# mrnorman/miniWeatherML

Hardware: AMD Instinct MI355X
Metric: cell-updates/s (higher is better)
Workload: dtype f64; 1 GPU; supercell 400x400x100 nens=1 per GPU (global 400x400x100, dx = dy = 500 m), WENO-FV dycore only, 3 tracers, CFL dt; parallelism=1x1 slab, halo_transport=none, V=8, strict=0, weno_order=5, schedule=one stream, schedule_code=4, y_faces_in_one_launch=True, zero_tracer_shortcut=True, zero_stores_skipped=True, zero_row_maps=True, alg_bytes_per_cell_update=512, alg_bytes_per_cell_update_boundary=768

## Files before the change

include/mw_cdna4.h:

```cpp
#ifndef MW_CDNA4_H
#define MW_CDNA4_H

#ifdef __cplusplus
extern "C" {
#endif

#define MW_NUM_STATE 5
#define MW_MAX_TRACERS 16

enum { MW_DATA_THERMAL = 0, MW_DATA_SUPERCELL = 1, MW_DATA_CITY = 2, MW_DATA_BUILDING = 3 };
enum { MW_BC_PERIODIC = 0, MW_BC_OPEN = 1, MW_BC_WALL = 2 };

typedef struct {
  int nz, ny, nx, nens, num_tracers;
  long long nx_glob, ny_glob, i_beg, j_beg;
  double xlen, ylen, zlen;
  int px, py, nproc_x, nproc_y;
  int neigh[9];
  int bc_x, bc_y, bc_z;
  int use_immersed, enable_gravity;
  int idWV;
  double R_d, R_v, cp_d, cp_v, p0, grav, gamma_d, kappa_d, C0, earthrot, latitude;
} mw_grid_t;

// ... 40 lines not shown

int  mw_weno5_edges(long long n, const double *stencils, double *edges, int strict, void *stream);
int  mw_strict_pow(long long n, const double *x, const double *y, double *out, unsigned char *main_path, void *stream);

int  mw_calib_copy(const double *in, double *out, long long n, void *stream);

int  mw_calib_fma64(int waves_per_simd, double seconds, double *out5, void *stream);
long long mw_calib_stage_arith_threads(long long cells, int levels);
int  mw_calib_stage_arith(const double *tab, int nlev, long long cells, int levels, int active_tracers, const double *bg4, double *sink, double *out3, void *stream);
int  mw_debug_spin(long long usec, void *stream);
long long mw_debug_launched_kernels(char *buf, long long cap, int reset);
long long mw_debug_zero_maps(mw_dycore_t h, unsigned int *out_host, long long cap_words, int *dims2);
long long mw_debug_zero_violations(mw_dycore_t h, unsigned long long *out4);
long long mw_debug_vapour_redo(mw_dycore_t h);
long long mw_debug_tracer_flags(mw_dycore_t h, unsigned char *out_host, long long cap);

int  mw_perturb_temperature(const mw_grid_t *g, double *temp, void *stream);
int  mw_perturb_temperature_random(const mw_grid_t *g, double *temp, void *stream);

int  mw_exchange_plan(const mw_grid_t *g, int *peers, int *send_order, int *recv_order, int *active);
typedef int (*mw_exchange_fn)(void *ctx, const double *sendW, const double *sendE, const double *sendS,
                              const double *sendN, double *recvW, double *recvE, double *recvS, double *recvN,
                              long long nWE, long long nSN, void *stream);
int  mw_dycore_set_exchange(mw_dycore_t h, mw_exchange_fn fn, void *ctx);
int  mw_rccl_unique_id(unsigned char *id128);
int  mw_dycore_use_rccl(mw_dycore_t h, const unsigned char *id128, int nranks, int myrank);
int  mw_dycore_use_rccl_self(mw_dycore_t h);
const char *mw_rccl_library_path(int *version);
int  mw_dycore_rccl_info(mw_dycore_t h, int *comm_ranks, int *comm_rank, int *lanes);
int  mw_dycore_rccl_allreduce_sum(void *dycore_handle, double *buf, long long n, void *stream);
// ... 155 lines not shown
```

miniweatherml_amd/capi.py:

```python
import ctypes as C
import os

_HERE = os.path.dirname(os.path.abspath(__file__))
LIB_PATH = os.environ.get("MW_LIB_PATH") or os.path.join(_HERE, "libmw_cdna4.so")

MW_MAX_TRACERS = 16
MW_SURROGATE_MAX_MODELS = 256
MW_ROLLOUT_MAX_MEMBERS = 30
MW_COMMITTEE_MAX_MODELS = 16
MW_RAIN_MAX_FIELDS, MW_RAIN_MAX_THRESHOLDS = 4, 8
DATA_THERMAL, DATA_SUPERCELL, DATA_CITY, DATA_BUILDING = 0, 1, 2, 3
BC_PERIODIC, BC_OPEN, BC_WALL = 0, 1, 2
INIT_IDS = {"thermal": DATA_THERMAL, "supercell": DATA_SUPERCELL, "city": DATA_CITY, "building": DATA_BUILDING}


class Grid(C.Structure):
    _fields_ = [
        ("nz", C.c_int), ("ny", C.c_int), ("nx", C.c_int), ("nens", C.c_int), ("num_tracers", C.c_int),
        ("nx_glob", C.c_longlong), ("ny_glob", C.c_longlong), ("i_beg", C.c_longlong), ("j_beg", C.c_longlong),
        ("xlen", C.c_double), ("ylen", C.c_double), ("zlen", C.c_double),
        ("px", C.c_int), ("py", C.c_int), ("nproc_x", C.c_int), ("nproc_y", C.c_int),
        ("neigh", C.c_int * 9),
        ("bc_x", C.c_int), ("bc_y", C.c_int), ("bc_z", C.c_int),
        ("use_immersed", C.c_int), ("enable_gravity", C.c_int),
# ... 25 lines not shown
    "mw_dycore_set_bc": (C.c_int, [C.c_void_p, C.c_int, C.c_int, C.c_int]),
    "mw_dycore_set_strict": (C.c_int, [C.c_void_p, C.c_int]),
    "mw_dycore_set_order": (C.c_int, [C.c_void_p, C.c_int]),
    "mw_dycore_set_option": (C.c_int, [C.c_void_p, C.c_char_p, C.c_longlong]),
    "mw_dycore_get_option": (C.c_int, [C.c_void_p, C.c_char_p, C.POINTER(C.c_longlong)]),
    "mw_build_flags": (C.c_int, []),
    "mw_calib_fma64": (C.c_int, [C.c_int, C.c_double, C.POINTER(C.c_double), C.c_void_p]),
    "mw_calib_stage_arith_threads": (C.c_longlong, [C.c_longlong, C.c_int]),
    "mw_calib_stage_arith": (C.c_int, [C.c_void_p, C.c_int, C.c_longlong, C.c_int, C.c_int, C.POINTER(C.c_double), C.c_void_p, C.POINTER(C.c_double), C.c_void_p]),
    "mw_debug_spin": (C.c_int, [C.c_longlong, C.c_void_p]),
    "mw_debug_launched_kernels": (C.c_longlong, [C.c_char_p, C.c_longlong, C.c_int]),
    "mw_debug_zero_maps": (C.c_longlong, [C.c_void_p, C.c_void_p, C.c_longlong, C.POINTER(C.c_int)]),
    "mw_debug_zero_violations": (C.c_longlong, [C.c_void_p, C.POINTER(C.c_ulonglong)]),
    "mw_debug_vapour_redo": (C.c_longlong, [C.c_void_p]),
    "mw_debug_tracer_flags": (C.c_longlong, [C.c_void_p, C.c_void_p, C.c_longlong]),
    "mw_dycore_path": (C.c_char_p, [C.c_void_p]),
    "mw_dycore_use_rccl_self": (C.c_int, [C.c_void_p]),
    "mw_rccl_selftest_config": (C.c_int, [C.c_int, C.c_int]),
    "mw_dycore_time_step": (C.c_int, [C.c_void_p] + [C.c_void_p] * 5 + [C.POINTER(C.c_void_p), C.c_double]),
    "mw_dycore_compute_tendencies": (C.c_int, [C.c_void_p] + [C.c_void_p] * 5 + [C.POINTER(C.c_void_p), C.c_double,
                                                                               C.c_void_p, C.c_void_p]),
    "mw_dycore_get_fluxes": (C.c_int, [C.c_void_p, C.POINTER(C.c_void_p)]),
    "mw_dycore_get_etime": (C.c_double, [C.c_void_p]),
    "mw_dycore_schedule": (C.c_int, [C.c_void_p]),
    "mw_dycore_rccl_info": (C.c_int, [C.c_void_p, C.POINTER(C.c_int), C.POINTER(C.c_int), C.POINTER(C.c_int)]),
    "mw_dycore_rccl_allreduce_sum": (C.c_int, [C.c_void_p, C.c_void_p, C.c_longlong, C.c_void_p]),
    "mw_dycore_rccl_bcast": (C.c_int, [C.c_void_p, C.c_void_p, C.c_longlong, C.c_int, C.c_void_p]),
    "mw_dycore_profile": (C.c_int, [C.c_void_p, C.c_int]),
    "mw_dycore_profile_get": (C.c_int, [C.c_void_p, C.c_int, C.POINTER(C.c_double), C.POINTER(C.c_longlong)]),
    "mw_calib_copy": (C.c_int, [C.c_void_p, C.c_void_p, C.c_longlong, C.c_void_p]),
# ... 142 lines not shown
```

miniweatherml_amd/csrc/mw_dycore.hip:

```cpp
#include "mw_dycore_int.h"
#include "mw_weno.h"
#include <map>
#include <set>
#include <tuple>
#include <mutex>
#include <cmath>
#include <cstring>

namespace mw {
static std::mutex g_launch_mu;
static std::set<const void *> g_launched;
void note_launch(const void *fn) { std::lock_guard<std::mutex> lk(g_launch_mu); g_launched.insert(fn); }

__global__ __launch_bounds__(256) void k_coupler_to_state(DyP p, CouplerPtrs c, double *__restrict__ S) {
#pragma clang fp contract(off)
  long long t = (long long)blockIdx.x * 256 + threadIdx.x;
  int k = blockIdx.y;
  int NXI = p.nx * p.nens;
  if (t >= (long long)p.ny * NXI) return;
  int j = (int)(t / NXI), ie = (int)(t - (long long)j * NXI);
  int e = ie % p.nens;
  long long ci = ((long long)k * p.ny + j) * NXI + ie;
  double rho_d = c.rho_d[ci], u = c.u[ci], v = c.v[ci], w = c.w[ci], temp = c.temp[ci];
  double rho_v = c.tr[p.idWV][ci];
// ... 807 lines not shown
namespace {
struct OptDesc { const char *key; int DyOpts::*field; long long lo, hi; int build; };
const OptDesc OPTS[] = {
  {"overlap", &DyOpts::overlap, -1, 1, 0}, {"pipe", &DyOpts::pipe, 0, 1, 0}, {"pipe_edge_inline", &DyOpts::pipe_edge_inline, 0, 1, 0},
  {"pipe_convert", &DyOpts::pipe_convert, 0, 1, 0}, {"pipe_split_edges", &DyOpts::pipe_split_edges, 0, 1, 0}, {"spec", &DyOpts::spec, 0, 1, 0}, {"wrap", &DyOpts::wrap, 0, 1, 0},
  {"y_all", &DyOpts::y_all, 0, 1, 0}, {"y_all_conv", &DyOpts::y_all_conv, 0, 1, 0}, {"member_major", &DyOpts::member_major, 0, 1, 0},
  {"mm_direct", &DyOpts::mm_direct, 0, 1, 0}, {"mm_conv", &DyOpts::mm_conv, 0, 1, 0}, {"fused_convert", &DyOpts::fused_convert, 0, 1, 0},
  {"fused_convert_mm", &DyOpts::fused_convert_mm, 0, 1, 0}, {"chunk_y", &DyOpts::chunk_y, 0, 1 << 20, 0}, {"chunk_yt", &DyOpts::chunk_yt, 0, 1 << 20, 0},
  {"chunk_z", &DyOpts::chunk_z, 0, 1 << 20, 0}, {"chunk_f", &DyOpts::chunk_f, 0, 1 << 20, 0}, {"chunk_model", &DyOpts::chunk_model, 0, 1, 0},
  {"tf_rows4", &DyOpts::tf_rows4, 0, 1, 0}, {"zero_skip", &DyOpts::zero_skip, 0, 1, 0}, {"zero_rows", &DyOpts::zero_rows, 0, 1, 0}, {"zero_stores", &DyOpts::zero_stores, 0, 1, 0}, {"zero_verify", &DyOpts::zero_verify, 0, 1, 0}, {"pipe_maps_early", &DyOpts::pipe_maps_early, 0, 1, 0}, {"rccl_lanes", &DyOpts::rccl_lanes, 0, 2, 0}, {"rccl_two_comms", &DyOpts::rccl_two_comms, -1, 1, 0},
  {"xchg_fuzz", &DyOpts::xchg_fuzz, 0, 0x7fffffff, 0}, {"rccl_prio", &DyOpts::rccl_prio, 0, 1, 0}, {"rccl_inline", &DyOpts::rccl_inline, 0, 1, 0},
  {"debug_no_patch", &DyOpts::debug_no_patch, 0, 1, 0},
};
struct OptDesc2 { const char *key; int DyOpts::*field; };
const OptDesc2 OPTS_VAPOUR[] = {{"vapour_state", &DyOpts::vapour_state}, {"debug_vapour_redo", &DyOpts::debug_vapour_redo}};
constexpr int BUILD_FLAGS = 0;
}
int mw_build_flags(void) { return BUILD_FLAGS; }
int mw_dycore_set_option(mw_dycore_t d, const char *key, long long value) {
  if (!d || !key) MW_FAIL("mw_dycore_set_option: null argument");
  if (!strcmp(key, "fused_tracers")) {
    if (value != 0 && value != 1) MW_FAIL("option fused_tracers must be 0 or 1");
    if (value && !(d->g.num_tracers <= 4 && d->g.nens <= 12)) MW_FAIL("option fused_tracers = 1 needs at most 4 tracers and 12 members");
    d->fused = (int)value;
    return 0;
  }
  for (const OptDesc2 &od : OPTS_VAPOUR) {
    if (strcmp(key, od.key)) continue;
    if (value != 0 && value != 1) MW_FAIL(std::string("option ") + key + " must be 0 or 1");
    d->o.*(od.field) = (int)value;
    return 0;
  }
  for (const OptDesc &od : OPTS) {
    if (strcmp(key, od.key)) continue;
    if (value < od.lo || value > od.hi) MW_FAIL(std::string("option ") + key + ": value out of range [" + std::to_string(od.lo) + ", " + std::to_string(od.hi) + "]");
    d->o.*(od.field) = (int)value;
    if (!strncmp(key, "chunk_", 6)) d->chunk_y = d->chunk_yt = d->chunk_z = d->chunk_f = 0;
    return 0;
  }
  MW_FAIL(std::string("unknown option: ") + key);
}
int mw_dycore_get_option(mw_dycore_t d, const char *key, long long *value) {
  if (!d || !key || !value) MW_FAIL("mw_dycore_get_option: null argument");
  if (!strcmp(key, "fused_tracers")) { *value = d->fused; return 0; }
  for (const OptDesc2 &od : OPTS_VAPOUR) if (!strcmp(key, od.key)) { *value = d->o.*(od.field); return 0; }
  for (const OptDesc &od : OPTS) if (!strcmp(key, od.key)) { *value = d->o.*(od.field); return 0; }
  MW_FAIL(std::string("unknown option: ") + key);
}
int mw_dycore_set_order(mw_dycore_t d, int ord) {
  if (!d) MW_FAIL("null handle");
  if (ord != 3 && ord != 5 && ord != 7 && ord != 9) MW_FAIL("WENO order must be 3, 5, 7 or 9");
  const int hs = (ord - 1) / 2, hx = std::max(HXc, hs + 1), hz = std::max(HZc, hs);
  const int old_ord = d->ord, old_hx = d->hxw, old_hz = d->hzw;
  auto rollback = [&]() { d->ord = old_ord; d->hxw = old_hx; d->hzw = old_hz; fill_params(d); return 1; };
  d->ord = ord; d->hxw = hx; d->hzw = hz;
  fill_params(d);
  if (!d->strides_ok) { set_error("mw_dycore_set_order: with this order's halo a variable of the block has more than 2^31 - 1 elements"); return rollback(); }
  if (check_halo_fit(d)) return rollback();
  if (hx != old_hx || hz != old_hz) {
    MW_HIP(hipStreamSynchronize(d->stream));
// ... 315 lines not shown
```

miniweatherml_amd/csrc/mw_dycore_int.h:

```cpp
#pragma once
#include "mw_common.h"
#include "mw_zero_rows.h"
#include <string>
#include <vector>
#include <algorithm>

#pragma GCC visibility push(hidden)

namespace mw { void note_launch(const void *fn); }
#define MW_KLAUNCH(kern, ...) do { mw::note_launch((const void *)&kern); hipLaunchKernelGGL(kern, __VA_ARGS__); } while (0)

using namespace mw;

struct DyOpts {
  int overlap = -1;
  int pipe = 1;
  int pipe_edge_inline = 0;
  int pipe_convert = 1;
  int pipe_split_edges = 1;
  int spec = 1;
  int wrap = 1;
  int y_all = 1, y_all_conv = 1;
  int member_major = 1, mm_direct = 1, mm_conv = 1;
  int fused_convert = 1, fused_convert_mm = 1;
  int chunk_y = 0, chunk_yt = 0, chunk_z = 0, chunk_f = 0;
  int chunk_model = 1;
  int tf_rows4 = 1;
  int zero_skip = 1;
  int zero_rows = 1;
  int pipe_maps_early = 1;
  int zero_stores = 1;
  int zero_verify = 0;
  int rccl_lanes = 0, rccl_two_comms = -1;
  int rccl_prio = 1;
  int rccl_inline = 1;
  int xchg_fuzz = 0;
  int debug_no_patch = 0;
  int vapour_state = 1;
  int debug_vapour_redo = 0;
};

struct mw_dycore_s {
  mw_grid_t g;
  DyOpts o;
  unsigned char pos[MW_MAX_TRACERS], adds[MW_MAX_TRACERS];
  DyP p;
  bool strides_ok = true;
  int ord = 5;
  int hxw = HXc, hzw = HZc;
  double etime = 0;
  int strict = 0;
  int last_march = 0;
  std::string path;
  double *S0 = nullptr, *S1 = nullptr, *S2 = nullptr, *S3 = nullptr;
// ... 99 lines not shown
```

miniweatherml_amd/csrc/mw_march.h:

```cpp
#pragma once
#include "mw_zero_rows.h"
#ifndef MW_XCD_SWIZZLE
#define MW_XCD_SWIZZLE 1
#endif

namespace mw {

__device__ __forceinline__ double shfl_from(double v, int src_lane) { return __shfl(v, src_lane, 64); }

__device__ __forceinline__ double fast_rcp(double x) {
#pragma clang fp contract(fast)
  double r = __builtin_amdgcn_rcp(x);
  r = r + r * (1.0 - x * r);
  r = r + r * (1.0 - x * r);
  return r;
}

#define MW_SCHED_FENCE() __builtin_amdgcn_sched_barrier(0)

template <int N>
__device__ __forceinline__ void landed(double (&a)[N]) {
#pragma unroll
  for (int i = 0; i < N; i++) asm volatile("" : "+v"(a[i]));
}
// ... 742 lines not shown
  return qnew;
}
__device__ __forceinline__ double tr_times(double a, double b) {
#pragma clang fp contract(off)
  return a * b;
}
__device__ __forceinline__ double tr_d13_temp(double press, double rho_dry, double rho_v, double R_d, double R_v) {
#pragma clang fp contract(off)
  return press / (rho_dry * R_d + rho_v * R_v);
}
struct XzVap {
  const double *FY;
  double *cq;
  double *crho, *ctemp;
  unsigned *redo;
};


template <int STAGE, bool N1, int MODE, int HPL, int K, int ORD, bool MT = false, bool VAP = false>
__global__ __launch_bounds__(256, 2) void k_xz_state(DyP p, const double *__restrict__ S, const double *__restrict__ Sn,
                                                  double *__restrict__ Sout, double *__restrict__ MX, double *__restrict__ MZ,
                                                  unsigned char *__restrict__ UPX, unsigned char *__restrict__ UPZ,
                                                  const double *__restrict__ tendY, double dt_stage, double dt_dyn, int chunk,
                                                  int tiles_x, double *__restrict__ cu, double *__restrict__ cv, double *__restrict__ cw,
                                                  MemberOff mo, XzVap va) {
  static_assert(!MT || (N1 && HPL && MODE == 1), "the member-co-located form is the D13 variant of the nens == 1 kernel");
  static_assert(!VAP || (N1 && HPL && K == 1 && !MT && ORD == 5), "the vapour form exists for the folded supercell configuration with nens == 1, WENO-5");
  constexpr int HS = (ORD - 1) / 2;
  const int wv = __builtin_amdgcn_readfirstlane((int)(threadIdx.x >> 6));
  int mt_e = 0, mt_sub = 0;
  if (MT) {
    mt_e = wv & (mo.n - 1); mt_sub = wv >> mo.sh;
    S += mt_e * mo.slab; Sn += mt_e * mo.slab; Sout += mt_e * mo.slab; MX += mt_e * mo.mx; UPX += mt_e * mo.mx; MZ += mt_e * mo.mz; UPZ += mt_e * mo.mz;
    tendY += mt_e * mo.tend; p.hypk += mt_e * mo.per; p.ce = mt_e;
  }
  __shared__ double lds_c[8];
  __shared__ double lds_xpart[5][256], lds_fzprev[5][256];
  extern __shared__ double lds_hp_all[];
  Segment sg;
  block_segment(chunk, p.nz, sg);
  const XzGeom g = xz_geom<N1, ORD>(p, sg.col, sg.a, sg.b, tiles_x, 0, MT ? mt_sub : -1, MT ? 4 >> mo.sh : 4);
  const int seg_len = sg.b - sg.a;
  double *lds_hp = lds_hp_all + (MT ? wv * (seg_len + 2) * 8 : 0);
// ... 12 lines not shown
  double *lds_q = lds_hp_all + (chunk + 2) * 8 + threadIdx.x;
  const int n = g.n, lane = g.lane, NXI = g.NXI, j = g.j, q = g.q, e = g.e;
  const double *col = S + (long long)(j + p.HY) * p.sJ + (long long)p.HX * n + g.qa;
  const long long cell0 = (long long)j * NXI + g.qc;
  const long long slab0 = (long long)(j + p.HY) * p.sJ + (long long)p.HX * n + g.qc;
  const int planeC = p.ny * NXI;
  double w[5][ORD], nxt[5], ct[5];
#pragma unroll
  for (int v = 0; v < 5; v++) {
    ct[v] = 0; lds_fzprev[v][threadIdx.x] = 0; lds_xpart[v][threadIdx.x] = 0;
#pragma unroll
    for (int s = 0; s < ORD; s++) w[v][s] = load_zlevel<K>(p, col + (long long)v * p.sV, g.kstart - HS + s, v == idW);
  }
  const bool vzq_on = VAP && MODE == 1 && (p.zq != nullptr) && p.zero_skip;
  unsigned vzseg = 0;
  if (VAP && MODE == 1) { const int tx_ = (q + (HS + 1) - lane) ; vzseg = zr_seg_mask(tx_ - (HS + 2), tx_ - (HS + 1) + 63 + 1, NXI, p.wrap_x != 0); }
  unsigned long long vlean_mask = 0ull;
  auto vlean_fetch = [&](int kc0) __attribute__((always_inline)) {
    const unsigned wz = p.zq[(long long)min(kc0 + lane + 2, p.nz - 1) * p.zq_ld + j + MW_ZR_HALO];
    vlean_mask = __ballot((wz & vzseg) == 0u);
  };
  if (VAP && MODE == 1 && vzq_on) vlean_fetch(g.ka);
  double wq[ORD], nxtq = 0, ctq = 0;
  int qr = (g.kstart - HS + ORD) % ORD;
#define MW_QSLOT(s_) (lds_q[(5 + ((qr + (s_)) >= ORD ? qr + (s_) - ORD : qr + (s_))) * 256])
  if (VAP) {
    lds_q[0] = 0; lds_q[256] = 0; lds_q[512] = 0; lds_q[768] = 0; lds_q[1024] = 0;
#pragma unroll
    for (int s = 0; s < ORD; s++) wq[s] = load_zlevel<K>(p, col + (long long)5 * p.sV, g.kstart - HS + s, false);
  }
#pragma unroll
  for (int v = 0; v < 5; v++) landed(w[v]);
  if (VAP) landed(wq);
  if (VAP) {
#pragma unroll
    for (int s = 0; s < ORD; s++) MW_QSLOT(s) = wq[s];
  }
  for (int k = g.kstart; k <= g.kb; k++) {
    const bool top = (k == p.nz);
    const bool xwork = (k >= g.ka) && (k < g.kb);
    const bool zface = (k >= g.ka);
    const bool fin = (k > g.ka);
    bool vlean = false;
    if (VAP && MODE == 1 && vzq_on) {
      const int ic = max(k - 1, g.ka) - g.ka;
      if (ic > 0 && (ic & 63) == 0) vlean_fetch(g.ka + ic);
      vlean = (vlean_mask >> (ic & 63)) & 1ull;
    }
    {
      const int kn = min(k + HS + 1, p.nz + p.HZ - 1);
#pragma unroll
      for (int v = 0; v < 5; v++) nxt[v] = load_zlevel<K>(p, col + (long long)v * p.sV, kn, v == idW);
      if (VAP) nxtq = load_zlevel<K>(p, col + (long long)5 * p.sV, kn, false);
    }
    double snv[5], tyv[5], immv = 0;
    const int kfc = max(k - 1, g.ka), kxc = min(max(k, g.ka), g.kb - 1);
#pragma unroll
    for (int l = 0; l < 5; l++) { snv[l] = 0; tyv[l] = 0; }
    if (STAGE != 1) {
#pragma unroll
      for (int l = 0; l < 5; l++) snv[l] = Sn[(long long)l * p.sV + slab0 + (long long)(kfc + p.HZ) * p.sK];
    }
// ... 89 lines not shown
        for (int s = 0; s < ORD; s++) wq[s] = MW_QSLOT(s);
        double beq; weno_window_edges<ORD>(wq, beq, teq); fzq = fs.m_upw * (up ? beq : ctq);
      }
      upz = up;
    }
    landed(nxt); landed(snv); landed(tyv); landed(immv);
    if (VAP) {
      landed(nxtq); landed(qnv); landed(fysq); landed(fynq);
      if (!top) MW_QSLOT(0) = nxtq;
      if (xwork) {
        const double feq = from_east<N1>(fxq, lane, n);
        lds_q[(k & 1) * 256] = tr_partial_xy(feq, fxq, fynq, fysq, lds_c[0], lds_c[4]);
        lds_q[(2 + (k & 1)) * 256] = tr_out_xy(tr_out_pair(feq, fxq, lds_c[0]), tr_out_pair(fynq, fysq, lds_c[4]));
      }
    }
    if (xwork && g.owns_face && (g.owns_cell || q >= NXI)) {
      const long long fo = (long long)k * p.fxK + (long long)j * p.fxJ + q;
      MX[fo] = fxs[idR];  UPX[fo] = (unsigned char)upx;
    }
    if (zface && g.owns_cell) {
      const long long fo = (long long)k * p.fzK + (long long)j * p.fzJ + q;
      MZ[fo] = fzs[idR];  UPZ[fo] = (unsigned char)upz;
    }
    if (fin) {
      const int kc = k - 1;
      const double hyc = HPL ? lds_hp[(kc - g.kstart) * 8] : p.hypk[(long long)(kc * n + e) * 8];
      constexpr int wi = HS - 1;
      const double rho_s = w[idR][wi] + hyc;
      const double rho_n = (STAGE == 1) ? rho_s : snv[idR] + hyc;
      double imm_coef = 0;
      if (Cf<K>::immersed(p)) { double tau = 1.e3 * dt_stage; imm_coef = -fmin(1.0, dt_stage / tau); }
      const double ru_s = w[idU][wi] * rho_s, rv_s = w[idV][wi] * rho_s;
      double inv_rho_new = 1.0;
      double *so = Sout + slab0 + (long long)(kc + p.HZ) * p.sK;
      double xpart[5], fzprev[5];
// ... 15 lines not shown
        if (l == idV && Cf<K>::sim2d(p)) tend = 0;
        if (Cf<K>::immersed(p)) { double imm_tend = imm_coef * q_s / dt_stage; tend = immv * imm_tend + (1 - immv) * tend; }
        double qnew;
        const double cdt = HPL ? lds_c[2] : (STAGE == 1) ? dt_dyn : (STAGE == 2) ? (1.0 / 4.0) * dt_dyn : (2.0 / 3.0) * dt_dyn;
        if (STAGE == 1)      qnew = q_n + cdt * tend;
        else if (STAGE == 2) qnew = (3.0 / 4.0) * q_n + (1.0 / 4.0) * q_s + cdt * tend;
        else                 qnew = (1.0 / 3.0) * q_n + (2.0 / 3.0) * q_s + cdt * tend;
        if (l == idR) inv_rho_new = fast_rcp(qnew + hyc);
        if (VAP && MODE == 1 && l == idR) rho_new_q = qnew + hyc;
        double stored = (l == idR || l == idT) ? qnew : qnew * inv_rho_new;
        if (MODE == 1 && l == idT) {
          const double *hq = HPL ? lds_hp + (kc - g.kstart) * 8 : p.hypk + (long long)(kc * n + e) * 8;
          stored = pressure_fast<K>(p, qnew, hq[1], hq[2], hq[3]);
          if (VAP) press_q = stored;
        }
        if (g.owns_cell && !(MODE == 1 && (l == idU || l == idV || l == idW))) so[(long long)l * p.sV] = stored;
        if (MODE == 1 && g.owns_cell && (l == idU || l == idV || l == idW))
          (l == idU ? cu : l == idV ? cv : cw)[cpl(p, cell0 + (long long)kc * planeC)] = stored;
      }
      if (VAP) {
        const double qs_raw = MW_QSLOT(wi);
        const double mass_available = tr_mass_available(qs_raw, rho_s);
        const double mass_out = tr_mass_out(oxyq, tr_out_pair(fzq, fzpq, lds_c[1]), lds_c[5]);
        if (__builtin_expect(g.owns_cell && mass_out > mass_available, 0)) *va.redo = 1u;
        const double q_s = tr_times(qs_raw, rho_s);
        const double q_n = (STAGE == 1) ? q_s : tr_times(qnv, rho_n);
        const double qnew = tr_combine<STAGE>(q_n, q_s, tr_tend(Pq, fzq, fzpq, lds_c[1]), lds_c[2], true);
        if (g.owns_cell) {
          if (MODE == 0) so[(long long)5 * p.sV] = tr_times(qnew, inv_rho_new);
          else           va.cq[cpl(p, cell0 + (long long)kc * planeC)] = qnew;
          if (MODE == 1 && vlean) {
// ... 205 lines not shown
    c.temp[ci] = press / (rho_dry * p.R_d + rho_v * p.R_v);
  }
}

template <int STAGE, int MODE, int T, bool N1, int K, int ORD, bool MT = false, int VS = 0>
__global__ __launch_bounds__(256, 2) void k_tracers_fused(DyP p, const double *__restrict__ S, const double *__restrict__ Sn, double *Sout,
                                                       const double *__restrict__ FY, const double *__restrict__ MX,
                                                       const double *__restrict__ MZ, const unsigned char *__restrict__ UPX,
                                                       const unsigned char *__restrict__ UPZ, double *__restrict__ DS,
                                                       double *__restrict__ DN, unsigned char *__restrict__ flags, unsigned int *__restrict__ dirty,
                                                       double dt, double dt_dyn, CouplerPtrs c, int chunk, int tiles_x, int rows4, MemberOff mo,
                                                       unsigned *vr, int vslot) {
  static_assert(N1 || ORD == 5, "the neighbour-load form exists for WENO-5 only");
  static_assert(!VS || (N1 && K == 1 && T == 3 && !MT && ORD == 5), "the form without the vapour exists for the folded supercell configuration with nens == 1, WENO-5");
  bool vredo = true;
  if (VS) {
    vredo = __builtin_amdgcn_readfirstlane((int)vr[vslot]) != 0;
    if (blockIdx.x == 0 && blockIdx.y == 0 && threadIdx.x == 0) { vr[(vslot + 1) & 7] = 0u; if (vredo) atomicAdd(&vr[8], 1u); }
  }
  static_assert(!MT || (N1 && MODE == 1), "the member-co-located form (see MemberOff) is the D13 variant of the nens == 1 kernel");
  constexpr int HS = (ORD - 1) / 2;
  const int wv = __builtin_amdgcn_readfirstlane((int)(threadIdx.x >> 6));
  int mt_e = 0, mt_sub = 0;
  if (MT) {
    mt_e = wv & (mo.n - 1); mt_sub = wv >> mo.sh;
    S += mt_e * mo.slab; Sn += mt_e * mo.slab; Sout += mt_e * mo.slab; FY += mt_e * mo.fy; MX += mt_e * mo.mx; UPX += mt_e * mo.mx;
    MZ += mt_e * mo.mz; UPZ += mt_e * mo.mz; DS += mt_e * mo.fx; DN += mt_e * mo.fz; flags += mt_e * mo.cells;
    p.hyc += mt_e * mo.per; p.ce = mt_e;
  }
  const int n = N1 ? 1 : p.nens;
  constexpr int t0 = 0;
// ... 40 lines not shown
  const int k_lo = max(ka - 1, 0);
  const int k_hi = min(kb, p.nz - 1);
  const int kstart = max(ka - 2, 0);
#if MW_ZERO_SKIP
  if (VS && !vredo && (p.zq != nullptr) && p.zero_skip && kb + 1 - kstart < 64) {
    const unsigned zseg_ = zr_seg_mask(tx * U - (hw + 1) * n, tx * U - hw * n + 63 + n, NXI, p.wrap_x != 0);
    const int kit = kstart + lane;
    const bool in_it = kit <= kb + 1, st_it = (kit - 2 >= ka) && (kit - 2 < kb);
    bool busy = in_it && (p.zq[(long long)min(kit, p.nz - 1) * p.zq_ld + j + MW_ZR_HALO] & zseg_) != 0u;
    const unsigned *zc_ = (MODE == 1) ? p.zqc : p.zqp;
    if (zc_ != nullptr) {
      const int kq_ = (MODE == 1) ? min(max(kit - 2, ka), kb - 1) : min(kit, p.nz - 1);
      busy = busy || (st_it && (zc_[(long long)kq_ * p.zq_ld + j + MW_ZR_HALO] & zseg_) != 0u);
    } else busy = true;
    if (!__any(busy)) {
      if (upd && do_y) for (int kp = ka; kp < kb; kp++) flags[(long long)(kp * p.ny + j) * NXI + q] = (unsigned char)0;
      return;
    }
  }
#endif
  double w[T][ORD], nxt[T], ct[T];
  double fxp[T], fzp[T], multp[T], szf[T], P[T];
  double wkm2[T];
  double rhos2 = 0;

#pragma unroll
  for (int v = 0; v < T; v++) {
    ct[v] = 0; fxp[v] = fzp[v] = szf[v] = P[v] = 0; multp[v] = 1; wkm2[v] = 0;
#pragma unroll
    for (int s = 0; s < ORD; s++) w[v][s] = load_zlevel(p, col + (long long)v * p.sV, kstart - HS + s, false);
  }
// ... 337 lines not shown
```

miniweatherml_amd/csrc/mw_march_sched.hip:

```cpp
#include "mw_dycore_int.h"
#include "mw_weno.h"
#define MW_MARCH_SCHED_KERNELS
#include "mw_march.h"

template <int STAGE, int MODE>
static int rk_stage_march(mw_dycore_s *d, double *Sin, const double *Sn, double *Sout, double dt_stage, double dt_dyn,
                          const CouplerPtrs &c) {
  const long long gs = d->gstage++;
  const int par = (int)(gs & 1), slot = (int)(gs & 7);
  hipStream_t ss = d->stream, ts = d->overlap ? d->tstream : d->stream;
  const int T = d->p.nt;
  zero_rows_stage(d, STAGE);
  ProfScope stage_scope(d, 8, ss);
  if (d->overlap && gs >= 2) MW_HIP(hipStreamWaitEvent(ss, d->ev_tr[(gs - 2) & 7], 0));
  if (halo_fill(d, Sin, 0, 5, ss, 0, true)) return 1;
  const bool conv = (STAGE == 1) && d->conv_pending;
  d->conv_pending = false;
  const bool mm_conv_ok = d->mm_direct && d->o.mm_conv && marching_config(d, view(d, 0).p) != 0;
  const bool yall = y_all_ok(d) && !(conv && ((d->member_major && !mm_conv_ok) || !d->o.y_all_conv));
  if (STAGE == 1) { if (conv) zero_rows_conv(d, Sin, false, ss); else zero_rows_forget(d, Sin); }
  if (STAGE == 3 && MODE == 0) zero_rows_forget(d, Sout);
  const bool vap = yall && d->o.vapour_state && d->fused && !d->overlap && !d->member_major && d->p.nens == 1 && d->ord == 5 && marching_config(d, d->p) == 1;
  const int vap_slot = vap ? slot : -1;
  {
// ... 151 lines not shown
    MW_KLAUNCH(k_coupler_to_state_fast, s ? plane_grid(nstrip, p.nz) : cgrid, dim3(256), 0, d->stream, p, c, d->S0, ylo, yhi, s ? 1 : 0);
  }
  MW_LAUNCH_CHECK();
  return 0;
}

extern "C" {
long long mw_debug_tracer_flags(mw_dycore_t d, unsigned char *out_host, long long cap) {
  if (!d || !d->flags) return -1;
  (void)hipStreamSynchronize(d->stream);
  if (d->tstream) (void)hipStreamSynchronize(d->tstream);
  const long long n = (long long)d->p.nC;
  if (out_host && cap > 0 && hipMemcpy(out_host, d->flags, (size_t)std::min(n, cap), hipMemcpyDeviceToHost) != hipSuccess) return -1;
  return n;
}
long long mw_debug_vapour_redo(mw_dycore_t d) {
  if (!d || !d->dirty) return -1;
  (void)hipStreamSynchronize(d->stream);
  if (d->tstream) (void)hipStreamSynchronize(d->tstream);
  unsigned int n = 0;
  if (hipMemcpy(&n, d->dirty + MW_VREDO_RING + 8, sizeof(n), hipMemcpyDeviceToHost) != hipSuccess) return -1;
  return (long long)n;
}
}
```

miniweatherml_amd/csrc/mw_march_tracers.hip:

```cpp
#include "mw_dycore_int.h"
#include "mw_weno.h"
#include "mw_march.h"

template <int T, bool N1>
static void launch_xz_tracers_t(mw_dycore_s *d, const double *S, dim3 grid, int chunk, int tiles_x, int t0, int par, double dt, int rows4,
                                hipStream_t st) {
  MW_KLAUNCH((k_xz_tracers<T, N1>), grid, dim3(256), 0, st, d->p, S, d->FX, d->FY, d->FZ, d->M[par][0], d->M[par][2], d->UP[par][0],
                     d->UP[par][2], dt, chunk, tiles_x, t0, rows4);
}

int launch_xz_tracers(mw_dycore_s *d, const double *S, int par, double dt, hipStream_t st) {
  const DyP &p = d->p;
  ProfScope ps(d, 7, st);
  dim3 grid; int chunk, tiles_x;
  if (xz_grid(d, p, grid, chunk, tiles_x)) return 1;
  const int rows4 = p.ny >= 4 ? 1 : 0;
  if (rows4) grid.x = (unsigned)(((p.ny + 3) / 4) * tiles_x);
  for (int t0 = 0; t0 < p.nt; t0 += 4) {
    int cnt = std::min(4, p.nt - t0);
    if (p.nens == 1) {
      switch (cnt) { case 1: launch_xz_tracers_t<1, true>(d, S, grid, chunk, tiles_x, t0, par, dt, rows4, st); break;
                     case 2: launch_xz_tracers_t<2, true>(d, S, grid, chunk, tiles_x, t0, par, dt, rows4, st); break;
                     case 3: launch_xz_tracers_t<3, true>(d, S, grid, chunk, tiles_x, t0, par, dt, rows4, st); break;
                     default: launch_xz_tracers_t<4, true>(d, S, grid, chunk, tiles_x, t0, par, dt, rows4, st); break; }
// ... 11 lines not shown
template <int STAGE, int MODE>
int launch_tracer_update(mw_dycore_s *d, const double *Sstar, const double *Sn, double *Sout, double dt_dyn, const CouplerPtrs &c,
                                hipStream_t st) {
  ProfScope ps(d, 2, st);
  const DyP &p = d->p;
  dim3 grid = plane_grid((long long)p.ny * p.nx * p.nens, p.nz);
  MW_KLAUNCH((k_tracer_update<STAGE, MODE>), grid, dim3(256), 0, st, p, Sstar, Sn, Sout, d->FX, d->FY, d->FZ, dt_dyn, c);
  MW_LAUNCH_CHECK();
  return 0;
}

template <int STAGE, int MODE, int T, bool N1, int K, int ORD = 5, int VS = 0>
static void launch_tracers_fused_t(mw_dycore_s *d, const View &v, const double *S, const double *Sn, double *Sout, dim3 grid, int chunk, int tiles_x, int par,
                                   double dt, double dt_dyn, const CouplerPtrs &c, int rows4, hipStream_t st, int vap_slot) {
  const int e = v.e;
  MW_KLAUNCH((k_tracers_fused<STAGE, MODE, T, N1, K, ORD, false, VS>), grid, dim3(256), 0, st, v.p, v.S(S), v.S(Sn), v.S(Sout), d->FY + e * v.f[1],
                     d->M[par][0] + e * v.m[0], d->M[par][2] + e * v.m[2], d->UP[par][0] + e * v.m[0], d->UP[par][2] + e * v.m[2],
                     d->FX + e * v.f[0], d->FZ + e * v.f[2], d->flags + e * v.cells, d->dirty + (d->fused_launches & 1), dt, dt_dyn, c, chunk, tiles_x, rows4, MemberOff(),
                     VS ? d->dirty + MW_VREDO_RING : nullptr, VS ? vap_slot : 0);
}
template <int STAGE, int MODE>
int launch_tracers_fused(mw_dycore_s *d, const double *S, const double *Sn, double *Sout, int par, double dt, double dt_dyn,
                                const CouplerPtrs &c, hipStream_t st, int vap_slot) {
  {
    ProfScope ps(d, 7, st);
    bool direct = false;
    if constexpr (STAGE == 3 && MODE == 1) direct = d->mm_direct;
    if constexpr (STAGE == 3 && MODE == 1) if (direct) {
      const View v = view(d, 0);
      const DyP &p = v.p;
      const MemberOff mo = member_off(d);
      const int U = 64 - 2 * ((d->ord - 1) / 2 + 1), tiles_x = (p.nx + U - 1) / U, rpb = 4 / mo.n;
      const long long waves = (long long)p.ny * tiles_x;
      const int chunk = d->chunk_f ? d->chunk_f : (d->chunk_f = balanced_chunk(d, p.nz, waves, d->o.chunk_f, 10000, 2, 4.5, true));
// ... 64 lines not shown
```

miniweatherml_amd/csrc/mw_march_xz.hip:

```cpp
#include "mw_dycore_int.h"
#include "mw_weno.h"
#include "mw_march.h"

int xz_grid(mw_dycore_s *d, const DyP &p, dim3 &grid, int &chunk, int &tiles_x) {
  int U = xz_cells_per_wave(p.nens, d->ord);
  if (U < 4) MW_FAIL("nens too large for the 64-lane x tiling (need nens <= 30)");
  tiles_x = (p.nx * p.nens + U - 1) / U;
  long long waves = (long long)p.ny * tiles_x;
  if (!d->chunk_z) {
    d->chunk_z = balanced_chunk(d, p.nz, waves, d->o.chunk_z, 10000, 2, 2.5, true);
    d->chunk_z = std::min(d->chunk_z, 900);
  }
  chunk = d->chunk_z;
  grid = dim3((unsigned)((waves + 3) / 4), (unsigned)((p.nz + chunk - 1) / chunk));
  return 0;
}

template <int STAGE, int MODE>
int launch_xz_state(mw_dycore_s *d, const double *S, const double *Sn, double *Sout, double dt_stage, double dt_dyn, int par,
                           const CouplerPtrs &c, int vap_slot) {
  ProfScope ps(d, 0);
  if constexpr (STAGE == 3 && MODE == 1) {
    if (d->mm_direct) {
      const View v = view(d, 0);
// ... 16 lines not shown
      return 0;
    }
  }
  for (int e = 0; e < n_views(d); e++) {
    const View v = view(d, e);
    const DyP &p = v.p;
    dim3 grid; int chunk, tiles_x;
    if (xz_grid(d, p, grid, chunk, tiles_x)) return 1;
    double *MX = d->M[par][0] + e * v.m[0], *MZ = d->M[par][2] + e * v.m[2], *tY = d->tendY + e * v.tend;
    unsigned char *UX = d->UP[par][0] + e * v.m[0], *UZ = d->UP[par][2] + e * v.m[2];
#define MW_XZ(N1_, HPL_, K_, O_, lds) MW_KLAUNCH((k_xz_state<STAGE, N1_, MODE, HPL_, K_, O_>), grid, dim3(256), (lds), d->stream, p, v.S(S), v.S(Sn), v.S(Sout), \
                                                 MX, MZ, UX, UZ, tY, dt_stage, dt_dyn, chunk, tiles_x, c.u, c.v, c.w, MemberOff(), XzVap())
#define MW_XZ_K(K_) { if (d->ord == 3) MW_XZ(true, 1, K_, 3, hpl_bytes); else MW_XZ(true, 1, K_, 5, hpl_bytes); }
    const size_t hpl_bytes = (size_t)(chunk + 2) * 64;
    if (vap_slot >= 0) {
      const XzVap va = {d->FY + (long long)5 * p.fyV, c.tr[0], c.rho_d, c.temp, d->dirty + MW_VREDO_RING + vap_slot};
      const size_t lds = hpl_bytes + (size_t)(5 + 5) * 256 * sizeof(double);
      MW_KLAUNCH((k_xz_state<STAGE, true, MODE, 1, 1, 5, false, true>), grid, dim3(256), lds, d->stream, p, v.S(S), v.S(Sn), v.S(Sout),
                 MX, MZ, UX, UZ, tY, dt_stage, dt_dyn, chunk, tiles_x, c.u, c.v, c.w, MemberOff(), va);
      if (d->o.debug_vapour_redo) MW_HIP(hipMemsetAsync(d->dirty + MW_VREDO_RING + vap_slot, 0xFF, sizeof(unsigned int), d->stream));
    } else
    if (p.nens == 1) {
      switch (marching_config(d, p)) { case 1: MW_XZ_K(1) break; case 2: MW_XZ_K(2) break; default: MW_XZ_K(0) break; }
    } else MW_XZ(false, 0, 0, 5, 0);
#undef MW_XZ_K
#undef MW_XZ
    MW_LAUNCH_CHECK();
  }
  return 0;
}

template int launch_xz_state<1, 0>(mw_dycore_s *, const double *, const double *, double *, double, double, int, const CouplerPtrs &, int);
template int launch_xz_state<2, 0>(mw_dycore_s *, const double *, const double *, double *, double, double, int, const CouplerPtrs &, int);
template int launch_xz_state<3, 0>(mw_dycore_s *, const double *, const double *, double *, double, double, int, const CouplerPtrs &, int);
template int launch_xz_state<3, 1>(mw_dycore_s *, const double *, const double *, double *, double, double, int, const CouplerPtrs &, int);
// ... 1 lines not shown
```

Measured before the change: 3.720 billion cell-updates/s.

## Skip face-flux and state stores in zero regions with lean-store handoff

Adds a default-on lean_stores option. The vapour xz kernel now consults the zero-row maps and skips writing x/z face fluxes and selected state entries in rows that are entirely zero. A second launch with lean=2 then runs only when the vapour-redo flag is set, to refill what was skipped. The fused tracer kernel also skips zeroing its flags when the previous dirty word shows everything was zero. The aim is to cut global store traffic, at the cost of an extra kernel launch and some correctness risk in the handoff, which a new debug poison routine is meant to test.

```diff
diff --git a/include/mw_cdna4.h b/include/mw_cdna4.h
--- a/include/mw_cdna4.h
+++ b/include/mw_cdna4.h
@@ -78,6 +78,7 @@
 long long mw_debug_zero_violations(mw_dycore_t h, unsigned long long *out4);
 long long mw_debug_vapour_redo(mw_dycore_t h);
 long long mw_debug_tracer_flags(mw_dycore_t h, unsigned char *out_host, long long cap);
+int  mw_debug_poison_handoff(mw_dycore_t h);
 
 int  mw_perturb_temperature(const mw_grid_t *g, double *temp, void *stream);
 int  mw_perturb_temperature_random(const mw_grid_t *g, double *temp, void *stream);
diff --git a/miniweatherml_amd/capi.py b/miniweatherml_amd/capi.py
--- a/miniweatherml_amd/capi.py
+++ b/miniweatherml_amd/capi.py
@@ -63,6 +63,7 @@
     "mw_debug_zero_violations": (C.c_longlong, [C.c_void_p, C.POINTER(C.c_ulonglong)]),
     "mw_debug_vapour_redo": (C.c_longlong, [C.c_void_p]),
     "mw_debug_tracer_flags": (C.c_longlong, [C.c_void_p, C.c_void_p, C.c_longlong]),
+    "mw_debug_poison_handoff": (C.c_int, [C.c_void_p]),
     "mw_dycore_path": (C.c_char_p, [C.c_void_p]),
     "mw_dycore_use_rccl_self": (C.c_int, [C.c_void_p]),
     "mw_rccl_selftest_config": (C.c_int, [C.c_int, C.c_int]),
diff --git a/miniweatherml_amd/csrc/mw_dycore.hip b/miniweatherml_amd/csrc/mw_dycore.hip
--- a/miniweatherml_amd/csrc/mw_dycore.hip
+++ b/miniweatherml_amd/csrc/mw_dycore.hip
@@ -845,6 +845,7 @@
 };
 struct OptDesc2 { const char *key; int DyOpts::*field; };
 const OptDesc2 OPTS_VAPOUR[] = {{"vapour_state", &DyOpts::vapour_state}, {"debug_vapour_redo", &DyOpts::debug_vapour_redo}};
+const OptDesc2 OPTS_LEAN[] = {{"lean_stores", &DyOpts::lean_stores}};
 constexpr int BUILD_FLAGS = 0;
 }
 int mw_build_flags(void) { return BUILD_FLAGS; }
@@ -856,10 +857,10 @@
     d->fused = (int)value;
     return 0;
   }
-  for (const OptDesc2 &od : OPTS_VAPOUR) {
-    if (strcmp(key, od.key)) continue;
+  for (const OptDesc2 *od : {&OPTS_VAPOUR[0], &OPTS_VAPOUR[1], &OPTS_LEAN[0]}) {
+    if (strcmp(key, od->key)) continue;
     if (value != 0 && value != 1) MW_FAIL(std::string("option ") + key + " must be 0 or 1");
-    d->o.*(od.field) = (int)value;
+    d->o.*(od->field) = (int)value;
     return 0;
   }
   for (const OptDesc &od : OPTS) {
@@ -875,6 +876,7 @@
   if (!d || !key || !value) MW_FAIL("mw_dycore_get_option: null argument");
   if (!strcmp(key, "fused_tracers")) { *value = d->fused; return 0; }
   for (const OptDesc2 &od : OPTS_VAPOUR) if (!strcmp(key, od.key)) { *value = d->o.*(od.field); return 0; }
+  for (const OptDesc2 &od : OPTS_LEAN) if (!strcmp(key, od.key)) { *value = d->o.*(od.field); return 0; }
   for (const OptDesc &od : OPTS) if (!strcmp(key, od.key)) { *value = d->o.*(od.field); return 0; }
   MW_FAIL(std::string("unknown option: ") + key);
 }
diff --git a/miniweatherml_amd/csrc/mw_dycore_int.h b/miniweatherml_amd/csrc/mw_dycore_int.h
--- a/miniweatherml_amd/csrc/mw_dycore_int.h
+++ b/miniweatherml_amd/csrc/mw_dycore_int.h
@@ -38,6 +38,7 @@
   int debug_no_patch = 0;
   int vapour_state = 1;
   int debug_vapour_redo = 0;
+  int lean_stores = 1;
 };
 
 struct mw_dycore_s {
diff --git a/miniweatherml_amd/csrc/mw_march.h b/miniweatherml_amd/csrc/mw_march.h
--- a/miniweatherml_amd/csrc/mw_march.h
+++ b/miniweatherml_amd/csrc/mw_march.h
@@ -780,6 +780,7 @@
   double *cq;
   double *crho, *ctemp;
   unsigned *redo;
+  int lean;
 };
 
 
@@ -793,6 +794,7 @@
   static_assert(!MT || (N1 && HPL && MODE == 1), "the member-co-located form is the D13 variant of the nens == 1 kernel");
   static_assert(!VAP || (N1 && HPL && K == 1 && !MT && ORD == 5), "the vapour form exists for the folded supercell configuration with nens == 1, WENO-5");
   constexpr int HS = (ORD - 1) / 2;
+  if (VAP && va.lean == 2 && *va.redo == 0u) return;
   const int wv = __builtin_amdgcn_readfirstlane((int)(threadIdx.x >> 6));
   int mt_e = 0, mt_sub = 0;
   if (MT) {
@@ -835,13 +837,27 @@
   }
   const bool vzq_on = VAP && MODE == 1 && (p.zq != nullptr) && p.zero_skip;
   unsigned vzseg = 0;
-  if (VAP && MODE == 1) { const int tx_ = (q + (HS + 1) - lane) ; vzseg = zr_seg_mask(tx_ - (HS + 2), tx_ - (HS + 1) + 63 + 1, NXI, p.wrap_x != 0); }
+  if (VAP && MODE == 1) { const int tx_ = __builtin_amdgcn_readfirstlane(q + (HS + 1) - lane); vzseg = zr_seg_mask(tx_ - (HS + 2), tx_ - (HS + 1) + 63 + 1, NXI, p.wrap_x != 0); }
   unsigned long long vlean_mask = 0ull;
   auto vlean_fetch = [&](int kc0) __attribute__((always_inline)) {
     const unsigned wz = p.zq[(long long)min(kc0 + lane + 2, p.nz - 1) * p.zq_ld + j + MW_ZR_HALO];
     vlean_mask = __ballot((wz & vzseg) == 0u);
   };
   if (VAP && MODE == 1 && vzq_on) vlean_fetch(g.ka);
+  const bool fst_on = VAP && va.lean == 1 && (p.zq != nullptr) && p.zero_skip;
+  unsigned fseg = 0;
+  if (fst_on) {
+    const int tx_ = __builtin_amdgcn_readfirstlane(q + (HS + 1) - lane), U_ = 64 - 2 * (HS + 1);
+    fseg = zr_seg_mask(tx_ - U_ - (HS + 2), tx_ + U_ - (HS + 1) + 63 + 1, NXI, p.wrap_x != 0);
+  }
+  unsigned long long fst_mask = ~0ull;
+  auto fst_fetch = [&](int kf0) __attribute__((always_inline)) {
+    const int kf = kf0 + lane;
+    const unsigned w0 = p.zq[(long long)min(max(kf - 1, 0), p.nz - 1) * p.zq_ld + j + MW_ZR_HALO];
+    const unsigned w1 = p.zq[(long long)min(kf, p.nz - 1) * p.zq_ld + j + MW_ZR_HALO];
+    fst_mask = __ballot(((w0 | w1) & fseg) != 0u);
+  };
+  if (fst_on) fst_fetch(g.ka);
   double wq[ORD], nxtq = 0, ctq = 0;
   int qr = (g.kstart - HS + ORD) % ORD;
 #define MW_QSLOT(s_) (lds_q[(5 + ((qr + (s_)) >= ORD ? qr + (s_) - ORD : qr + (s_))) * 256])
@@ -867,6 +883,12 @@
       const int ic = max(k - 1, g.ka) - g.ka;
       if (ic > 0 && (ic & 63) == 0) vlean_fetch(g.ka + ic);
       vlean = (vlean_mask >> (ic & 63)) & 1ull;
+    }
+    bool fst = true;
+    if (VAP) {
+      const int fi = max(k - g.ka, 0);
+      if (fst_on && fi > 0 && (fi & 63) == 0) fst_fetch(k);
+      fst = (fst_mask >> (fi & 63)) & 1ull;
     }
     {
       const int kn = min(k + HS + 1, p.nz + p.HZ - 1);
@@ -986,11 +1008,11 @@
         lds_q[(2 + (k & 1)) * 256] = tr_out_xy(tr_out_pair(feq, fxq, lds_c[0]), tr_out_pair(fynq, fysq, lds_c[4]));
       }
     }
-    if (xwork && g.owns_face && (g.owns_cell || q >= NXI)) {
+    if (xwork && fst && g.owns_face && (g.owns_cell || q >= NXI)) {
       const long long fo = (long long)k * p.fxK + (long long)j * p.fxJ + q;
       MX[fo] = fxs[idR];  UPX[fo] = (unsigned char)upx;
     }
-    if (zface && g.owns_cell) {
+    if (zface && fst && g.owns_cell) {
       const long long fo = (long long)k * p.fzK + (long long)j * p.fzJ + q;
       MZ[fo] = fzs[idR];  UPZ[fo] = (unsigned char)upz;
     }
@@ -1036,7 +1058,7 @@
           stored = pressure_fast<K>(p, qnew, hq[1], hq[2], hq[3]);
           if (VAP) press_q = stored;
         }
-        if (g.owns_cell && !(MODE == 1 && (l == idU || l == idV || l == idW))) so[(long long)l * p.sV] = stored;
+        if (g.owns_cell && !(MODE == 1 && (l == idU || l == idV || l == idW)) && !(VAP && MODE == 1 && vlean && fst_on)) so[(long long)l * p.sV] = stored;
         if (MODE == 1 && g.owns_cell && (l == idU || l == idV || l == idW))
           (l == idU ? cu : l == idV ? cv : cw)[cpl(p, cell0 + (long long)kc * planeC)] = stored;
       }
@@ -1272,7 +1294,10 @@
   static_assert(N1 || ORD == 5, "the neighbour-load form exists for WENO-5 only");
   static_assert(!VS || (N1 && K == 1 && T == 3 && !MT && ORD == 5), "the form without the vapour exists for the folded supercell configuration with nens == 1, WENO-5");
   bool vredo = true;
+  const unsigned int *dirty_prev = nullptr;
   if (VS) {
+    if (vslot >> 3) dirty_prev = ((vslot >> 3) == 1) ? dirty + 1 : dirty - 1;
+    vslot &= 7;
     vredo = __builtin_amdgcn_readfirstlane((int)vr[vslot]) != 0;
     if (blockIdx.x == 0 && blockIdx.y == 0 && threadIdx.x == 0) { vr[(vslot + 1) & 7] = 0u; if (vredo) atomicAdd(&vr[8], 1u); }
   }
@@ -1343,7 +1368,8 @@
       busy = busy || (st_it && (zc_[(long long)kq_ * p.zq_ld + j + MW_ZR_HALO] & zseg_) != 0u);
     } else busy = true;
     if (!__any(busy)) {
-      if (upd && do_y) for (int kp = ka; kp < kb; kp++) flags[(long long)(kp * p.ny + j) * NXI + q] = (unsigned char)0;
+      const bool all_zero = dirty_prev != nullptr && *dirty_prev == 0u;
+      if (!all_zero && upd && do_y) for (int kp = ka; kp < kb; kp++) flags[(long long)(kp * p.ny + j) * NXI + q] = (unsigned char)0;
       return;
     }
   }
diff --git a/miniweatherml_amd/csrc/mw_march_sched.hip b/miniweatherml_amd/csrc/mw_march_sched.hip
--- a/miniweatherml_amd/csrc/mw_march_sched.hip
+++ b/miniweatherml_amd/csrc/mw_march_sched.hip
@@ -189,6 +189,21 @@
   if (out_host && cap > 0 && hipMemcpy(out_host, d->flags, (size_t)std::min(n, cap), hipMemcpyDeviceToHost) != hipSuccess) return -1;
   return n;
 }
+int mw_debug_poison_handoff(mw_dycore_t d) {
+  if (!d || !d->S3) MW_FAIL("mw_debug_poison_handoff: null handle");
+  const DyP &p = d->p;
+  const size_t fn[3] = {(size_t)p.fxV, (size_t)p.fyV, (size_t)p.fzV};
+  for (int b = 0; b < 2; b++) for (int a = 0; a < 3; a += 2) {
+    MW_HIP(hipMemsetAsync(d->M[b][a], 0xFF, fn[a] * sizeof(double), d->stream));
+    MW_HIP(hipMemsetAsync(d->UP[b][a], 0xFF, fn[a], d->stream));
+  }
+  for (int e = 0; e < n_views(d); e++) {
+    const View v = view(d, e);
+    for (int l : {(int)idR, (int)idT}) MW_HIP(hipMemsetAsync(v.S(d->S3) + (long long)l * v.p.sV, 0xFF, (size_t)v.p.sV * sizeof(double), d->stream));
+  }
+  if (d->tstream) { MW_HIP(hipStreamSynchronize(d->stream)); }
+  return 0;
+}
 long long mw_debug_vapour_redo(mw_dycore_t d) {
   if (!d || !d->dirty) return -1;
   (void)hipStreamSynchronize(d->stream);
diff --git a/miniweatherml_amd/csrc/mw_march_tracers.hip b/miniweatherml_amd/csrc/mw_march_tracers.hip
--- a/miniweatherml_amd/csrc/mw_march_tracers.hip
+++ b/miniweatherml_amd/csrc/mw_march_tracers.hip
@@ -49,10 +49,11 @@
 static void launch_tracers_fused_t(mw_dycore_s *d, const View &v, const double *S, const double *Sn, double *Sout, dim3 grid, int chunk, int tiles_x, int par,
                                    double dt, double dt_dyn, const CouplerPtrs &c, int rows4, hipStream_t st, int vap_slot) {
   const int e = v.e;
+  const int prev_word = !d->o.lean_stores ? 0 : (d->fused_launches & 1) ? 2 : 1;
   MW_KLAUNCH((k_tracers_fused<STAGE, MODE, T, N1, K, ORD, false, VS>), grid, dim3(256), 0, st, v.p, v.S(S), v.S(Sn), v.S(Sout), d->FY + e * v.f[1],
                      d->M[par][0] + e * v.m[0], d->M[par][2] + e * v.m[2], d->UP[par][0] + e * v.m[0], d->UP[par][2] + e * v.m[2],
                      d->FX + e * v.f[0], d->FZ + e * v.f[2], d->flags + e * v.cells, d->dirty + (d->fused_launches & 1), dt, dt_dyn, c, chunk, tiles_x, rows4, MemberOff(),
-                     VS ? d->dirty + MW_VREDO_RING : nullptr, VS ? vap_slot : 0);
+                     VS ? d->dirty + MW_VREDO_RING : nullptr, VS ? vap_slot + 8 * prev_word : 0);
 }
 template <int STAGE, int MODE>
 int launch_tracers_fused(mw_dycore_s *d, const double *S, const double *Sn, double *Sout, int par, double dt, double dt_dyn,
diff --git a/miniweatherml_amd/csrc/mw_march_xz.hip b/miniweatherml_amd/csrc/mw_march_xz.hip
--- a/miniweatherml_amd/csrc/mw_march_xz.hip
+++ b/miniweatherml_amd/csrc/mw_march_xz.hip
@@ -54,11 +54,14 @@
 #define MW_XZ_K(K_) { if (d->ord == 3) MW_XZ(true, 1, K_, 3, hpl_bytes); else MW_XZ(true, 1, K_, 5, hpl_bytes); }
     const size_t hpl_bytes = (size_t)(chunk + 2) * 64;
     if (vap_slot >= 0) {
-      const XzVap va = {d->FY + (long long)5 * p.fyV, c.tr[0], c.rho_d, c.temp, d->dirty + MW_VREDO_RING + vap_slot};
+      XzVap va = {d->FY + (long long)5 * p.fyV, c.tr[0], c.rho_d, c.temp, d->dirty + MW_VREDO_RING + vap_slot, d->o.lean_stores ? 1 : 0};
       const size_t lds = hpl_bytes + (size_t)(5 + 5) * 256 * sizeof(double);
-      MW_KLAUNCH((k_xz_state<STAGE, true, MODE, 1, 1, 5, false, true>), grid, dim3(256), lds, d->stream, p, v.S(S), v.S(Sn), v.S(Sout),
-                 MX, MZ, UX, UZ, tY, dt_stage, dt_dyn, chunk, tiles_x, c.u, c.v, c.w, MemberOff(), va);
+#define MW_XZ_VAP() MW_KLAUNCH((k_xz_state<STAGE, true, MODE, 1, 1, 5, false, true>), grid, dim3(256), lds, d->stream, p, v.S(S), v.S(Sn), v.S(Sout), \
+                               MX, MZ, UX, UZ, tY, dt_stage, dt_dyn, chunk, tiles_x, c.u, c.v, c.w, MemberOff(), va)
+      MW_XZ_VAP();
       if (d->o.debug_vapour_redo) MW_HIP(hipMemsetAsync(d->dirty + MW_VREDO_RING + vap_slot, 0xFF, sizeof(unsigned int), d->stream));
+      if (va.lean && p.zq != nullptr && p.zero_skip) { MW_LAUNCH_CHECK(); va.lean = 2; MW_XZ_VAP(); }
+#undef MW_XZ_VAP
     } else
     if (p.nens == 1) {
       switch (marching_config(d, p)) { case 1: MW_XZ_K(1) break; case 2: MW_XZ_K(2) break; default: MW_XZ_K(0) break; }
```

Measured after the change: 3.800 billion cell-updates/s (median of 6 runs). 1.02x the previous value.
